# UltronAI/Depth-VO-Feat

Hardware: AMD Instinct MI355X
Metric: KITTI 256x832 stereo-seq samples/sec fwd+bwd (higher is better)
Workload: dtype f32

## Files before the change

### depth-vo-feat_amd/csrc/conv_head.hip

```cpp
#include "conv_head.h"
#include "conv_epilogue.h"

namespace {

using dvfp::apply_act;

constexpr int HT_W = 64, HT_H = 4;
constexpr int HP_W = HT_W + 2, HP_H = HT_H + 2;
constexpr int HCK = 8;

__device__ __forceinline__ void stage_tile(float *lds, const float *__restrict__ src, int64_t plane, int nch, int H, int W,
                                           int y0, int x0) {
    for (int e = threadIdx.x; e < nch * HP_H * HP_W; e += 256) {
        const int ch = e / (HP_H * HP_W), r = e - ch * (HP_H * HP_W), py = r / HP_W, px = r - py * HP_W;
        const int y = y0 + py - 1, x = x0 + px - 1;
        lds[e] = (y >= 0 && y < H && x >= 0 && x < W) ? src[ch * plane + (int64_t)y * W + x] : 0.f;
    }
}

template <int ROWS, int MO, class WK>
__device__ __forceinline__ void taps9(const float (&v)[ROWS + 2][3], WK wk, float (&acc)[ROWS][MO]) {
#pragma unroll
    for (int m = 0; m < MO; ++m)
#pragma unroll
        for (int k = 0; k < 9; ++k) {
            const float w = wk(m, k);
#pragma unroll
            for (int r = 0; r < ROWS; ++r) acc[r][m] = fmaf(w, v[k / 3 + r][k % 3], acc[r][m]);
        }
}

constexpr int FT_H = 8;
constexpr int HEAD_MAX_SEGS = 3;
struct HeadSegs {
    const float *p[HEAD_MAX_SEGS];
    int c[HEAD_MAX_SEGS];
    int n;
};
template <int MO, int HCKT, int FTH>
__global__ __launch_bounds__(256) void head_fwd_kernel(const HeadSegs in, const float *__restrict__ w,
                                                       const float *__restrict__ bias, float *__restrict__ out, int C, int H,
                                                       int W, int tilesX, int act, float alpha, float beta, int ws_m, int ws_c,
                                                       int flip, const float *__restrict__ mask) {
    constexpr int ROWS = FTH / 4, FPH = FTH + 2, FPN = FPH * HP_W, FLD = (FPN + 255) / 256;
    extern __shared__ __attribute__((aligned(16))) float wsh[];
    float *tile = wsh + ((MO * C * 9 + 3) & ~3);
    for (int e = threadIdx.x; e < MO * C * 9; e += 256) {
        const int m = e / (C * 9), r = e - m * (C * 9), c = r / 9, k = r - c * 9;
        const float wv = w[(int64_t)m * ws_m + (int64_t)c * ws_c + (flip ? 8 - k : k)];
        if (MO == 16) wsh[(c * MO + m) * 9 + k] = wv;
        else wsh[e] = wv;
    }
    const int n = blockIdx.y, tY = blockIdx.x / tilesX, tX = blockIdx.x - tY * tilesX;
    const int y0 = tY * FTH, x0 = tX * HT_W;
    const int lx = threadIdx.x & (HT_W - 1), ly = (threadIdx.x >> 6) * ROWS;
    const int64_t plane = (int64_t)H * W;
    int soff[FLD];
#pragma unroll
    for (int i = 0; i < FLD; ++i) {
        const int e = threadIdx.x + 256 * i, py = e / HP_W, px = e - py * HP_W;
        const int y = y0 + py - 1, x = x0 + px - 1;
        soff[i] = (e < FPN && y >= 0 && y < H && x >= 0 && x < W) ? y * W + x : -1;
    }
    float acc[ROWS][MO];
#pragma unroll
    for (int m = 0; m < MO; ++m)
#pragma unroll
        for (int r = 0; r < ROWS; ++r) acc[r][m] = bias ? bias[m] : 0.f;
    float stg[HCKT][FLD];
    static_assert(HEAD_MAX_SEGS == 3, "segment select below");
    auto seg_ptr = [&](int sg) { return sg == 0 ? in.p[0] : sg == 1 ? in.p[1] : in.p[2]; };
    auto seg_ch = [&](int sg) { return sg == 0 ? in.c[0] : sg == 1 ? in.c[1] : in.c[2]; };
    auto issue = [&](int sg, int cs) {
        const int sc = seg_ch(sg), nch = min(HCKT, sc - cs);
        const float *src = seg_ptr(sg) + ((int64_t)n * sc + cs) * plane;
#pragma unroll
        for (int ch = 0; ch < HCKT; ++ch)
#pragma unroll
            for (int i = 0; i < FLD; ++i) stg[ch][i] = (ch < nch && soff[i] >= 0) ? src[ch * plane + soff[i]] : 0.f;
    };
    issue(0, 0);
    int sg = 0, cs = 0, cg = 0;
    while (sg < in.n) {
        const int nch = min(HCKT, seg_ch(sg) - cs);
        int sg2 = sg, cs2 = cs + HCKT;
        if (cs2 >= seg_ch(sg)) { ++sg2; cs2 = 0; }
        __syncthreads();
#pragma unroll
        for (int ch = 0; ch < HCKT; ++ch)
#pragma unroll
            for (int i = 0; i < FLD; ++i) {
                const int e = threadIdx.x + 256 * i;
                if (e < FPN) tile[ch * FPN + e] = stg[ch][i];
            }
        __syncthreads();
        if (sg2 < in.n) issue(sg2, cs2);
        auto hood = [&](int ch, float (&v)[ROWS + 2][3]) __attribute__((always_inline)) {
            const float *t = tile + ch * FPN + ly * HP_W + lx;
#pragma unroll
            for (int a = 0; a < ROWS + 2; ++a)
#pragma unroll
                for (int b = 0; b < 3; ++b) v[a][b] = t[a * HP_W + b];
        };
        if constexpr (MO != 16) {
            auto wlds = [&](int c) __attribute__((always_inline)) {
                return [=](int m, int k) __attribute__((always_inline)) { return wsh[(m * C + c) * 9 + k]; };
            };
            float part[3][ROWS][MO];
#pragma unroll
            for (int q = 0; q < 3; ++q)
#pragma unroll
                for (int r = 0; r < ROWS; ++r)
#pragma unroll
                    for (int m = 0; m < MO; ++m) part[q][r][m] = 0.f;
            int ch = 0;
            for (; ch + 4 <= nch; ch += 4) {
                float v4[4][ROWS + 2][3];
#pragma unroll
                for (int q = 0; q < 4; ++q) hood(ch + q, v4[q]);
#pragma unroll
                for (int q = 0; q < 4; ++q)
#pragma unroll
                    for (int m = 0; m < MO; ++m) {
                        const float *wm = wsh + (m * C + cg + ch + q) * 9;
#pragma unroll
                        for (int k = 0; k < 9; ++k) {
                            const float wk = wm[k];
#pragma unroll
                            for (int r = 0; r < ROWS; ++r) {
                                if (q == 0) acc[r][m] = fmaf(wk, v4[q][k / 3 + r][k % 3], acc[r][m]);
                                else part[q - 1][r][m] = fmaf(wk, v4[q][k / 3 + r][k % 3], part[q - 1][r][m]);
                            }
                        }
                    }
            }
            for (; ch < nch; ++ch) {
                float v[ROWS + 2][3];
                hood(ch, v);
                taps9<ROWS, MO>(v, wlds(cg + ch), acc);
            }
#pragma unroll
            for (int r = 0; r < ROWS; ++r)
#pragma unroll
                for (int m = 0; m < MO; ++m) acc[r][m] += (part[0][r][m] + part[1][r][m]) + part[2][r][m];
        } else {
            for (int ch = 0; ch < nch; ++ch) {
                float v[ROWS + 2][3];
                hood(ch, v);
                typedef float f4h __attribute__((ext_vector_type(4)));
                const f4h *wq = reinterpret_cast<const f4h *>(wsh + (cg + ch) * (MO * 9));
                f4h wr[MO * 9 / 4];
#pragma unroll
                for (int q = 0; q < MO * 9 / 4; ++q) wr[q] = wq[q];
                taps9<ROWS, MO>(v, [&](int m, int k) __attribute__((always_inline)) { return wr[(m * 9 + k) >> 2][(m * 9 + k) & 3]; }, acc);
            }
        }
        cg += nch; sg = sg2; cs = cs2;
    }
    const int x = x0 + lx;
#pragma unroll
    for (int r = 0; r < ROWS; ++r) {
        const int y = y0 + ly + r;
        if (y < H && x < W) {
            if (mask) {
#pragma unroll
                for (int m = 0; m < MO; ++m) {
                    const int64_t idx = ((int64_t)n * MO + m) * plane + (int64_t)y * W + x;
                    out[idx] = mask[idx] > 0.f ? acc[r][m] : 0.f;
                }
            } else {
#pragma unroll
                for (int m = 0; m < MO; ++m)
                    out[((int64_t)n * MO + m) * plane + (int64_t)y * W + x] = apply_act(acc[r][m], act, alpha, beta);
            }
        }
    }
}

template <int MO>
__global__ __launch_bounds__(256) void head_dgrad_kernel(const float *__restrict__ dpre, const float *__restrict__ w,
                                                         float *__restrict__ din, int C, int H, int W, int tilesX,
                                                         const float *__restrict__ mask) {
    __shared__ float tile[MO * HP_H * HP_W];
    extern __shared__ __attribute__((aligned(16))) float wsh[];
    constexpr int WPC = (MO * 9 + 3) & ~3;
    for (int e = threadIdx.x; e < C * MO * 9; e += 256) {
        const int c = e / (MO * 9), r = e - c * (MO * 9), m = r / 9, k = r - m * 9;
        wsh[c * WPC + r] = w[((int64_t)m * C + c) * 9 + k];
    }
    const int n = blockIdx.y, tY = blockIdx.x / tilesX, tX = blockIdx.x - tY * tilesX;
    const int y0 = tY * HT_H, x0 = tX * HT_W;
    const int lx = threadIdx.x & (HT_W - 1), ly = threadIdx.x >> 6;
    const int64_t plane = (int64_t)H * W;
    stage_tile(tile, dpre + (int64_t)n * MO * plane, plane, MO, H, W, y0, x0);
    __syncthreads();
    float g[MO][9];
#pragma unroll
    for (int m = 0; m < MO; ++m)
#pragma unroll
        for (int a = 0; a < 3; ++a)
#pragma unroll
            for (int b = 0; b < 3; ++b) g[m][a * 3 + b] = tile[m * (HP_H * HP_W) + (ly + 2 - a) * HP_W + (lx + 2 - b)];
    const int y = y0 + ly, x = x0 + lx;
    if (y >= H || x >= W) return;
    const int64_t base = (int64_t)n * C * plane + (int64_t)y * W + x;
    float *dst = din + base;
    const float *mk = mask ? mask + base : nullptr;
    for (int c0 = 0; c0 < C; c0 += 4) {
        float sv[4], mv[4];
#pragma unroll
        for (int q = 0; q < 4; ++q) {
            const int c = min(c0 + q, C - 1);
            mv[q] = mk ? mk[c * plane] : 1.f;
            const float *wc = wsh + c * WPC;
            float s = 0.f;
#pragma unroll
            for (int m = 0; m < MO; ++m)
#pragma unroll
                for (int k = 0; k < 9; ++k) s = fmaf(wc[m * 9 + k], g[m][k], s);
            sv[q] = s;
        }
#pragma unroll
        for (int q = 0; q < 4; ++q)
            if (c0 + q < C) dst[(c0 + q) * plane] = (mv[q] > 0.f) ? sv[q] : 0.f;
    }
}

template <bool VEC>
__device__ __forceinline__ void hw_load4(const float *__restrict__ p, int x0, int W, bool ok, float (&v)[4]) {
    if (VEC) {
        typedef float f4 __attribute__((ext_vector_type(4)));
        f4 t = {0.f, 0.f, 0.f, 0.f};
        if (ok) t = *reinterpret_cast<const f4 *>(p);
#pragma unroll
        for (int j = 0; j < 4; ++j) v[j] = t[j];
    } else {
#pragma unroll
        for (int j = 0; j < 4; ++j) v[j] = (ok && x0 + j < W) ? p[j] : 0.f;
    }
}

template <int MO, int CCH, bool VEC>
__global__ __launch_bounds__(256) void head_wgrad_kernel(const float *__restrict__ in, const float *__restrict__ dpre,
                                                         float *dw, int C, int H, int W, int RS, int xgroups, int segs,
                                                         int64_t units, float *part = nullptr) {
    constexpr int A = CCH * 9 * MO;
    __shared__ float red[4 * A];
    const int c0 = blockIdx.x * CCH;
    const int64_t plane = (int64_t)H * W;
    const int upi = segs * xgroups;
    float acc[CCH][9][MO];
#pragma unroll
    for (int c = 0; c < CCH; ++c)
#pragma unroll
        for (int t = 0; t < 9; ++t)
#pragma unroll
            for (int m = 0; m < MO; ++m) acc[c][t][m] = 0.f;
    for (int64_t ub = blockIdx.y; ub * 256 < units; ub += gridDim.y) {
        const int64_t u = ub * 256 + threadIdx.x;
        const bool live = u < units;
        const int n = live ? (int)(u / upi) : 0, q = live ? (int)(u - (int64_t)n * upi) : 0;
        const int seg = q / xgroups, xg = q - seg * xgroups;
        const int y0 = seg * RS, y1 = min(H, y0 + RS), x0 = xg * 4;
        const float *ip = in + ((int64_t)n * C + c0) * plane + x0;
        const float *dp = dpre + (int64_t)n * MO * plane + x0;
        const bool lok = x0 > 0, rok = x0 + 4 < W;
        auto load_in = [&](int r, float (&x)[CCH][6]) __attribute__((always_inline)) {
            const bool ok = live && r >= 0 && r < H;
            const int64_t ro = (int64_t)r * W;
#pragma unroll
            for (int c = 0; c < CCH; ++c) {
                const bool okc = ok && c0 + c < C;
                const float *p = ip + c * plane + ro;
                float v[4];
                hw_load4<VEC>(p, x0, W, okc, v);
                x[c][0] = (okc && lok) ? p[-1] : 0.f;
#pragma unroll
                for (int j = 0; j < 4; ++j) x[c][1 + j] = v[j];
                x[c][5] = (okc && rok) ? p[4] : 0.f;
            }
        };
        auto load_dp = [&](int y, float (&g)[MO][4]) __attribute__((always_inline)) {
            const bool ok = live && y >= y0 && y < y1;
#pragma unroll
            for (int m = 0; m < MO; ++m) hw_load4<VEC>(dp + m * plane + (int64_t)y * W, x0, W, ok, g[m]);
        };
        float d[3][MO][4], dn[MO][4], xc[CCH][6], xn[CCH][6];
#pragma unroll
        for (int m = 0; m < MO; ++m)
#pragma unroll
            for (int j = 0; j < 4; ++j) d[0][m][j] = d[1][m][j] = 0.f;
        load_dp(y0, d[2]);
        load_in(y0 - 1, xc);
        for (int i = 0; i < RS + 2; ++i) {
            const int r = y0 - 1 + i;
            load_in(i + 1 < RS + 2 ? r + 1 : H, xn);
            load_dp(r + 2, dn);
#pragma unroll
            for (int c = 0; c < CCH; ++c)
#pragma unroll
                for (int ta = 0; ta < 3; ++ta)
#pragma unroll
                    for (int tb = 0; tb < 3; ++tb)
#pragma unroll
                        for (int m = 0; m < MO; ++m)
#pragma unroll
                            for (int j = 0; j < 4; ++j)
                                acc[c][ta * 3 + tb][m] = fmaf(d[2 - ta][m][j], xc[c][j + tb], acc[c][ta * 3 + tb][m]);
#pragma unroll
            for (int m = 0; m < MO; ++m)
#pragma unroll
                for (int j = 0; j < 4; ++j) { d[0][m][j] = d[1][m][j]; d[1][m][j] = d[2][m][j]; d[2][m][j] = dn[m][j]; }
#pragma unroll
            for (int c = 0; c < CCH; ++c)
#pragma unroll
                for (int j = 0; j < 6; ++j) xc[c][j] = xn[c][j];
        }
    }
    const int wave = threadIdx.x >> 6, lane = threadIdx.x & 63;
#pragma unroll
    for (int c = 0; c < CCH; ++c)
#pragma unroll
        for (int t = 0; t < 9; ++t)
#pragma unroll
            for (int m = 0; m < MO; ++m) {
                const float s = wave_sum(acc[c][t][m]);
                if (lane == 0) red[wave * A + (c * 9 + t) * MO + m] = s;
            }
    __syncthreads();
    const int a = threadIdx.x;
    if (a < A) {
        const int c = a / (9 * MO), q = a - c * (9 * MO), t = q / MO, m = q - t * MO;
        if (c0 + c < C) {
            const float s = (red[a] + red[A + a]) + (red[2 * A + a] + red[3 * A + a]);
            const int64_t o = ((int64_t)m * C + c0 + c) * 9 + t;
            if (part) part[(int64_t)blockIdx.y * MO * C * 9 + o] = s;
            else atomicAdd(&dw[o], s);
        }
    }
}

__global__ __launch_bounds__(256) void head_wgrad_finish_kernel(const float *__restrict__ part, float *dw, int n, int groups) {
    const int e = blockIdx.x * 256 + threadIdx.x;
    if (e >= n) return;
    float s = 0.f;
    for (int g = 0; g < groups; ++g) s += part[(int64_t)g * n + e];
    dw[e] += s;
}


template <int CO, int K>
__global__ __launch_bounds__(256) void dconvt_s2_fwd_kernel(const float *__restrict__ in, const float *__restrict__ w,
                                                            const float *__restrict__ bias, float *__restrict__ out, int C, int H,
                                                            int W, int OH, int OW, int act, float alpha, float beta) {
    extern __shared__ __attribute__((aligned(16))) float wlds[];
    constexpr int WPC = CO * K * K;
    static_assert(WPC % 4 == 0, "weights of one input channel are read in 16-byte pieces");
    typedef float f4w __attribute__((ext_vector_type(4)));
    for (int e = threadIdx.x; e < C * WPC / 4; e += 256)
        reinterpret_cast<f4w *>(wlds)[e] = reinterpret_cast<const f4w *>(w)[e];
    __syncthreads();
    const int x = blockIdx.x * 64 + (threadIdx.x & 63), y = blockIdx.y * 4 + (threadIdx.x >> 6), n = blockIdx.z;
    const bool inside = x < W && y < H;
    const bool rok[3] = {y - 1 >= 0 && y - 1 < H, y < H, y + 1 < H}, cok[3] = {x - 1 >= 0 && x - 1 < W, x < W, x + 1 < W};
    float acc[2][2][CO];
#pragma unroll
    for (int co = 0; co < CO; ++co) {
        const float b = bias ? bias[co] : 0.f;
        acc[0][0][co] = acc[0][1][co] = acc[1][0][co] = acc[1][1][co] = b;
    }
    const int64_t plane = (int64_t)H * W;
    const float *ip = in + (int64_t)n * C * plane + (int64_t)y * W + x;
    for (int ci = 0; ci < C; ++ci) {
        float v[3][3];
#pragma unroll
        for (int r = (K == 3 ? 1 : 0); r < 3; ++r)
#pragma unroll
            for (int c = (K == 3 ? 1 : 0); c < 3; ++c) v[r][c] = (rok[r] && cok[c]) ? ip[(r - 1) * W + (c - 1)] : 0.f;
        const f4w *wc = reinterpret_cast<const f4w *>(wlds + ci * WPC);
        f4w wq[WPC / 4];
#pragma unroll
        for (int q = 0; q < WPC / 4; ++q) wq[q] = wc[q];
#pragma unroll
        for (int co = 0; co < CO; ++co) {
#pragma unroll
            for (int a = 0; a < K; ++a) {
                const int dy = (a + 1) & 1;
                const int ry = 1 + ((dy + 1 - a) >> 1);
#pragma unroll
                for (int b = 0; b < K; ++b) {
                    const int dx = (b + 1) & 1;
                    const int rx = 1 + ((dx + 1 - b) >> 1);
                    const int f = co * K * K + a * K + b;
                    acc[dy][dx][co] = fmaf(wq[f >> 2][f & 3], v[ry][rx], acc[dy][dx][co]);
                }
            }
        }
        ip += plane;
    }
    if (!inside) return;
    const int64_t oplane = (int64_t)OH * OW;
    float *op = out + (int64_t)n * CO * oplane;
#pragma unroll
    for (int dy = 0; dy < 2; ++dy) {
        const int Y = 2 * y + dy;
        if (Y >= OH) continue;
        const int X = 2 * x;
#pragma unroll
        for (int co = 0; co < CO; ++co) {
            float r0 = apply_act(acc[dy][0][co], act, alpha, beta), r1 = apply_act(acc[dy][1][co], act, alpha, beta);
            float *q = op + co * oplane + (int64_t)Y * OW + X;
            if (X + 1 < OW && (OW & 1) == 0) {
                typedef float f2 __attribute__((ext_vector_type(2)));
                f2 t; t.x = r0; t.y = r1;
                *reinterpret_cast<f2 *>(q) = t;
            } else {
                if (X < OW) q[0] = r0;
                if (X + 1 < OW) q[1] = r1;
            }
        }
    }
}

}

bool dvf_head_applicable(const dvf_conv_desc *d, int nseg) {
    return nseg == 1 && !d->transposed && d->KH == 3 && d->KW == 3 && d->stride == 1 && d->pad == 1 && d->C_out >= 1 &&
           d->C_out <= 4 && d->H_out == d->H_in && d->W_out == d->W_in && d->C_in >= 4 && d->C_in * d->C_out <= 1024 &&
           dvf_tune("DVF_NO_HEAD") == nullptr;
}
bool dvf_head_fwd_applicable(const dvf_conv_desc *d, int nseg) {
    static const int maxc = dvf_tune("DVF_HEAD_FWD_MAXC") ? atoi(dvf_tune("DVF_HEAD_FWD_MAXC")) : 127;
    return dvf_head_applicable(d, nseg) && d->C_in <= maxc;
}
bool dvf_head_dgrad_applicable(const dvf_conv_desc *d, int nseg) {
    static const int maxc = dvf_tune("DVF_HEAD_DGRAD_MAXC") ? atoi(dvf_tune("DVF_HEAD_DGRAD_MAXC")) : 32;
    return dvf_head_applicable(d, nseg) && d->C_in <= maxc;
}

bool dvf_dconvt_applicable(const dvf_conv_desc *d, int nseg) {
    const bool k3 = d->KH == 3 && d->KW == 3, k4 = d->KH == 4 && d->KW == 4;
    return nseg == 1 && d->transposed && d->stride == 2 && d->pad == 1 && (k3 || k4) && d->C_out == 16 &&
           d->C_in >= 8 && d->C_in <= 64 && d->H_out <= 2 * d->H_in && d->W_out <= 2 * d->W_in &&
           (int64_t)d->H_in * d->W_in >= 64 * 64 && (int64_t)d->N * d->C_out * d->H_out * d->W_out < ((int64_t)1 << 31) &&
           dvf_tune("DVF_NO_DCONVT") == nullptr;
}

int dvf_dconvt_fwd(const dvf_conv_desc *d, const float *in, const float *w, const float *bias, float *out, hipStream_t st) {
    const dim3 grid(cdiv(d->W_in, 64), cdiv(d->H_in, 4), d->N);
    const size_t lds = (size_t)d->C_in * d->C_out * d->KH * d->KW * 4;
    if ((reinterpret_cast<uintptr_t>(w) & 15) != 0 || lds > 64 * 1024) return DVF_ERR_UNSUPPORTED;
#define DCONVT(CO, K) dconvt_s2_fwd_kernel<CO, K><<<grid, 256, lds, st>>>(in, w, bias, out, d->C_in, d->H_in, d->W_in, d->H_out, d->W_out, d->act, d->alpha, d->beta)
    if (d->KH == 3) DCONVT(16, 3);
    else DCONVT(16, 4);
#undef DCONVT
    DVF_LAUNCH_CHECK();
    dvf_note_head(DVF_K_DCONVT_FWD, d->C_out, d->KH);
    return DVF_OK;
}

#define HEAD_CASE(N, ...) case N: { constexpr int MO = N; __VA_ARGS__; } break;
#define HEAD_DISPATCH(MOV, CALL, ...)             \
    switch (MOV) {                               \
        HEAD_CASE(1, CALL) HEAD_CASE(2, CALL) HEAD_CASE(3, CALL) HEAD_CASE(4, CALL) __VA_ARGS__ \
        default: return DVF_ERR_UNSUPPORTED;     \
    }

static int head_fwd_launch(int MOv, const HeadSegs &in, const float *w, const float *bias, float *out, int C, int N, int H, int W,
                           int act, float alpha, float beta, int ws_m, int ws_c, int flip, const float *mask, hipStream_t st) {
    const bool lowres = (int64_t)N * H * W <= (int64_t)4 * 64 * 208 && MOv <= 4 && C >= 32;
    const int FTH = lowres ? 4 : FT_H, HCKT = lowres ? 32 : HCK;
    const int tilesX = cdiv(W, HT_W), tilesY = cdiv(H, FTH);
    const dim3 grid(tilesX * tilesY, N);
    const size_t lds = ((size_t)((MOv * C * 9 + 3) & ~3) + (size_t)HCKT * (FTH + 2) * HP_W) * 4;
#define HEAD_FWD_GO(HC, FH) head_fwd_kernel<MO, HC, FH><<<grid, 256, lds, st>>>(in, w, bias, out, C, H, W, tilesX, act, alpha, beta, ws_m, ws_c, flip, mask)
    if (lowres) {
        static bool big[5] = {false, false, false, false, false};
        HEAD_DISPATCH(MOv, {
            if (lds > 64 * 1024 && !big[MO]) {
                if (hipFuncSetAttribute(reinterpret_cast<const void *>(&head_fwd_kernel<MO, 32, 4>), hipFuncAttributeMaxDynamicSharedMemorySize, 160 * 1024) != hipSuccess) return DVF_ERR_LAUNCH;
                big[MO] = true;
            }
            HEAD_FWD_GO(32, 4); });
    } else {
        HEAD_DISPATCH(MOv, (HEAD_FWD_GO(8, 8)), HEAD_CASE(16, (HEAD_FWD_GO(8, 8))));
    }
#undef HEAD_FWD_GO
    DVF_LAUNCH_CHECK();
    return DVF_OK;
}

int dvf_head_fwd(const dvf_conv_desc *d, const float *in, const float *w, const float *bias, float *out, hipStream_t st) {
    const int one = d->C_in;
    return dvf_head_fwd_segs(d, &in, &one, 1, w, bias, out, st);
}

bool dvf_head_wide_applicable(const dvf_conv_desc *d, int nseg) {
    return nseg >= 1 && nseg <= HEAD_MAX_SEGS && !d->transposed && d->KH == 3 && d->KW == 3 && d->stride == 1 && d->pad == 1 &&
           d->C_out == 16 && d->C_in <= 24 && d->H_out == d->H_in && d->W_out == d->W_in &&
           (int64_t)d->H_in * d->W_in >= 64 * 64 && dvf_tune("DVF_NO_HEAD") == nullptr && dvf_tune("DVF_NO_WIDE_HEAD") == nullptr;
}

int dvf_head_fwd_segs(const dvf_conv_desc *d, const float *const *in_segs, const int *seg_channels, int nseg, const float *w,
                      const float *bias, float *out, hipStream_t st) {
    HeadSegs in{};
    for (int s = 0; s < HEAD_MAX_SEGS; ++s) { in.p[s] = s < nseg ? in_segs[s] : in_segs[0]; in.c[s] = s < nseg ? seg_channels[s] : 0; }
    in.n = nseg;
    const int rc = head_fwd_launch(d->C_out, in, w, bias, out, d->C_in, d->N, d->H_in, d->W_in, d->act, d->alpha, d->beta,
                                   d->C_in * 9, 9, 0, nullptr, st);
    if (rc) return rc;
    dvf_note_head(DVF_K_HEAD_FWD, d->C_out, nseg);
    return DVF_OK;
}

bool dvf_head_seg_dgrad_applicable(const dvf_conv_desc *d, int segc) {
    const bool narrow = segc >= 1 && segc <= 4 && d->C_out >= 4 && d->C_out * segc <= 1024;
    const bool wide = segc == 16 && d->C_out <= 24 && (int64_t)d->H_in * d->W_in >= 64 * 64 &&
                      dvf_tune("DVF_NO_WIDE_HEAD") == nullptr;
    return !d->transposed && d->KH == 3 && d->KW == 3 && d->stride == 1 && d->pad == 1 && (narrow || wide) &&
           d->H_out == d->H_in && d->W_out == d->W_in && dvf_tune("DVF_NO_HEAD") == nullptr;
}

int dvf_head_seg_dgrad(const dvf_conv_desc *d, const float *dpre, const float *w, float *din, int seg_off, int segc,
                       hipStream_t st, const float *mask) {
    const float *wseg = w + (int64_t)seg_off * 9;
    HeadSegs in{};
    for (int s = 0; s < HEAD_MAX_SEGS; ++s) { in.p[s] = dpre; in.c[s] = s == 0 ? d->C_out : 0; }
    in.n = 1;
    const int rc = head_fwd_launch(segc, in, wseg, nullptr, din, d->C_out, d->N, d->H_in, d->W_in, DVF_ACT_NONE, 1.f, 0.f, 9,
                                   d->C_in * 9, 1, mask, st);
    if (rc) return rc;
    dvf_note_head(DVF_K_HEAD_SEG_DGRAD, segc);
    return DVF_OK;
}

int dvf_head_dgrad(const dvf_conv_desc *d, const float *dpre, const float *w, float *din, hipStream_t st, const float *mask) {
    const int tilesX = cdiv(d->W_in, HT_W), tilesY = cdiv(d->H_in, HT_H);
    const dim3 grid(tilesX * tilesY, d->N);
    HEAD_DISPATCH(d->C_out, (head_dgrad_kernel<MO><<<grid, 256, (size_t)d->C_in * ((MO * 9 + 3) & ~3) * 4, st>>>(
                                dpre, w, din, d->C_in, d->H_in, d->W_in, tilesX, mask)));
    DVF_LAUNCH_CHECK();
    dvf_note_head(DVF_K_HEAD_DGRAD, d->C_out);
    return DVF_OK;
}

struct HeadWgradGrid { int cch, RS, xgroups, segs, chunks, groups; int64_t units; };
static HeadWgradGrid head_wgrad_grid(const dvf_conv_desc *d) {
    HeadWgradGrid g;
    g.xgroups = cdiv(d->W_in, 4);
    auto blocks = [&](int cch, int rs) {
        return (int64_t)cdiv(d->C_in, cch) * (((int64_t)d->N * cdiv(d->H_in, rs) * g.xgroups + 255) / 256);
    };
    const int min_blocks = 400, max_blocks = 1024;
    g.cch = (d->C_out <= 2 && blocks(4, 8) >= 512) ? 4 : 2;
    g.RS = 8;
    if (const char *t = dvf_tune("DVF_HEAD_WG_CCH")) g.cch = (atoi(t) == 4 && d->C_out <= 2) ? 4 : 2;
    while (g.RS > 2 && blocks(g.cch, g.RS) < min_blocks) g.RS >>= 1;
    if (const char *t = dvf_tune("DVF_HEAD_WG_RS")) g.RS = atoi(t) > 0 ? atoi(t) : g.RS;
    g.segs = cdiv(d->H_in, g.RS);
    g.units = (int64_t)d->N * g.segs * g.xgroups;
    g.chunks = cdiv(d->C_in, g.cch);
    const int64_t nub = (g.units + 255) / 256;
    int64_t groups = max_blocks / g.chunks;
    if (groups < 1) groups = 1;
    if (groups > nub) groups = nub;
    g.groups = (int)groups;
    return g;
}

int64_t dvf_head_wgrad_ws_floats(const dvf_conv_desc *d) {
    return (int64_t)head_wgrad_grid(d).groups * d->C_out * d->C_in * 9;
}

int dvf_head_wgrad(const dvf_conv_desc *d, const float *in, const float *dpre, float *dw, int accumulate, hipStream_t st,
                   float *ws, int64_t ws_floats) {
    if (!accumulate && hipMemsetAsync(dw, 0, sizeof(float) * (size_t)d->C_out * d->C_in * 9, st) != hipSuccess)
        return DVF_ERR_LAUNCH;
    const HeadWgradGrid g = head_wgrad_grid(d);
    const dim3 grid(g.chunks, g.groups);
    float *part = (ws && ws_floats >= dvf_head_wgrad_ws_floats(d)) ? ws : nullptr;
    const bool vec = d->W_in % 4 == 0 && ((reinterpret_cast<uintptr_t>(in) | reinterpret_cast<uintptr_t>(dpre)) & 15) == 0;
#define HEAD_WGRAD_GO(CCH, VEC) head_wgrad_kernel<MO, CCH, VEC><<<grid, 256, 0, st>>>(in, dpre, dw, d->C_in, d->H_in, d->W_in, g.RS, g.xgroups, g.segs, g.units, part)
    HEAD_DISPATCH(d->C_out, {
        if (MO <= 2 && g.cch == 4) { if (vec) HEAD_WGRAD_GO((MO <= 2 ? 4 : 2), true); else HEAD_WGRAD_GO((MO <= 2 ? 4 : 2), false); }
        else { if (vec) HEAD_WGRAD_GO(2, true); else HEAD_WGRAD_GO(2, false); } });
#undef HEAD_WGRAD_GO
    DVF_LAUNCH_CHECK();
    if (part) {
        const int n = d->C_out * d->C_in * 9;
        head_wgrad_finish_kernel<<<(n + 255) / 256, 256, 0, st>>>(part, dw, n, g.groups);
        DVF_LAUNCH_CHECK();
    }
    dvf_note_head(DVF_K_HEAD_WGRAD, d->C_out, part != nullptr);
    return DVF_OK;
}
```

Before: 663.5.

## Add MFMA kernels for stride-2 transposed conv and thin 16-output 3x3 conv

Adds an MFMA (16x16x4 f32 matrix-core) version of the stride-2 transposed convolution. It decomposes the output into four parity classes and double-buffers input and weight chunks through registers into LDS. It also adds a persistent-block MFMA kernel for 3x3 convolutions with 16 outputs and at most 24 input channels, which prefetches the next tile while computing the current one. The transposed-conv path is on by default when C_in is a multiple of 4, while the thin 3x3 path runs only when DVF_THIN_MFMA=1. The goal is to move the scalar FMA work onto matrix cores, at the cost of extra LDS staging and more code complexity.

```diff
diff --git a/depth-vo-feat_amd/csrc/conv_head.hip b/depth-vo-feat_amd/csrc/conv_head.hip
--- a/depth-vo-feat_amd/csrc/conv_head.hip
+++ b/depth-vo-feat_amd/csrc/conv_head.hip
@@ -422,6 +422,274 @@
     }
 }
 
+typedef float f4m __attribute__((ext_vector_type(4)));
+constexpr int TM_W = 64, TM_H = 4, TM_RS = TM_W + 2, TM_PN = (TM_H + 2) * TM_RS, TM_FLD = (TM_PN + 255) / 256;
+
+constexpr int T3_PS = TM_PN + 10;
+constexpr int T3_WLD = (24 * 9 * 16 + 255) / 256;
+constexpr int T3_BLOCKS = 4 * 256;
+template <int SC>
+__global__ __launch_bounds__(256) void thin3x3_mfma_kernel(const HeadSegs in, const float *__restrict__ w,
+                                                           const float *__restrict__ bias, float *__restrict__ out, int C, int H,
+                                                           int W, int tilesX, int tilesY, int total, int act, float alpha, float beta,
+                                                           int ws_m, int ws_c, int flip, const float *__restrict__ mask) {
+    extern __shared__ __attribute__((aligned(16))) float wsh[];
+    const int K = C * 9, NS = (K + 3) >> 2;
+    float *tile = wsh + NS * 64;
+    const int lane = threadIdx.x & 63, wave = threadIdx.x >> 6, g = lane >> 4, px = lane & 15;
+    const int64_t plane = (int64_t)H * W;
+    const int per = tilesX * tilesY;
+    static_assert(HEAD_MAX_SEGS == 3, "segment select below");
+    const int c01 = in.c[0] + in.c[1];
+    int soff[TM_FLD];
+    float stg[SC][TM_FLD];
+    auto issue = [&](int t) {
+        const int n = t / per, r = t - n * per, tY = r / tilesX, tX = r - tY * tilesX;
+#pragma unroll
+        for (int i = 0; i < TM_FLD; ++i) {
+            const int e = threadIdx.x + 256 * i, py = e / TM_RS, qx = e - py * TM_RS;
+            const int y = tY * TM_H + py - 1, x = tX * TM_W + qx - 1;
+            soff[i] = (e < TM_PN && y >= 0 && y < H && x >= 0 && x < W) ? y * W + x : -1;
+        }
+#pragma unroll
+        for (int ch = 0; ch < SC; ++ch) {
+            const int c = min(ch, C - 1), sg = (c >= in.c[0]) + (c >= c01);
+            const float *sp = sg == 0 ? in.p[0] : sg == 1 ? in.p[1] : in.p[2];
+            const int sc = sg == 0 ? in.c[0] : sg == 1 ? in.c[1] : in.c[2], first = sg == 0 ? 0 : sg == 1 ? in.c[0] : c01;
+            const float *src = sp + ((int64_t)n * sc + (c - first)) * plane;
+#pragma unroll
+            for (int i = 0; i < TM_FLD; ++i) stg[ch][i] = src[max(soff[i], 0)];
+        }
+    };
+    {
+        float wst[T3_WLD];
+#pragma unroll
+        for (int i = 0; i < T3_WLD; ++i) {
+            const int e = threadIdx.x + 256 * i, k = min(e >> 4, K - 1), m = e & 15, c = k / 9, t = k - c * 9;
+            wst[i] = 256 * i < NS * 64 ? w[(int64_t)m * ws_m + (int64_t)c * ws_c + (flip ? 8 - t : t)] : 0.f;
+        }
+        issue(blockIdx.x);
+#pragma unroll
+        for (int i = 0; i < T3_WLD; ++i) {
+            const int e = threadIdx.x + 256 * i;
+            if (e < NS * 64) wsh[e] = (e >> 4) < K ? wst[i] : 0.f;
+        }
+        if (C & 3)
+            for (int e = threadIdx.x; e < TM_PN; e += 256) tile[C * T3_PS + e] = 0.f;
+    }
+    int boff[9];
+#pragma unroll
+    for (int s = 0; s < 9; ++s) {
+        const int kl = 4 * s + g, cl = kl / 9, t = kl - cl * 9;
+        boff[s] = cl * T3_PS + (t / 3) * TM_RS + (t % 3);
+    }
+    float bv[4];
+#pragma unroll
+    for (int r = 0; r < 4; ++r) bv[r] = bias ? bias[4 * g + r] : 0.f;
+    for (int t = blockIdx.x; t < total; t += gridDim.x) {
+        __syncthreads();
+#pragma unroll
+        for (int ch = 0; ch < SC; ++ch)
+#pragma unroll
+            for (int i = 0; i < TM_FLD; ++i) {
+                const int e = threadIdx.x + 256 * i;
+                if (ch < C && e < TM_PN) tile[ch * T3_PS + e] = soff[i] >= 0 ? stg[ch][i] : 0.f;
+            }
+        __syncthreads();
+        if (t + (int)gridDim.x < total) issue(t + gridDim.x);
+        f4m acc[4];
+#pragma unroll
+        for (int r = 0; r < 4; ++r)
+#pragma unroll
+            for (int q = 0; q < 4; ++q) acc[q][r] = bv[r];
+        const float *tb = tile + wave * TM_RS + px, *wb = wsh + lane;
+        int s0 = 0;
+        for (; s0 + 9 <= NS; s0 += 9) {
+#pragma unroll
+            for (int s3 = 0; s3 < 9; s3 += 3) {
+                float a[3], b[3][4];
+#pragma unroll
+                for (int s = 0; s < 3; ++s) {
+                    a[s] = wb[(s3 + s) * 64];
+#pragma unroll
+                    for (int q = 0; q < 4; ++q) b[s][q] = tb[boff[s3 + s] + 16 * q];
+                }
+                __builtin_amdgcn_sched_barrier(0);
+#pragma unroll
+                for (int s = 0; s < 3; ++s)
+#pragma unroll
+                    for (int q = 0; q < 4; ++q) acc[q] = __builtin_amdgcn_mfma_f32_16x16x4f32(a[s], b[s][q], acc[q], 0, 0, 0);
+                __builtin_amdgcn_sched_barrier(0);
+            }
+            tb += 4 * T3_PS;
+            wb += 9 * 64;
+        }
+#pragma unroll
+        for (int s = 0; s < 8; ++s)
+            if (s0 + s < NS) {
+                const float a = wb[s * 64];
+                float b[4];
+#pragma unroll
+                for (int q = 0; q < 4; ++q) b[q] = tb[boff[s] + 16 * q];
+#pragma unroll
+                for (int q = 0; q < 4; ++q) acc[q] = __builtin_amdgcn_mfma_f32_16x16x4f32(a, b[q], acc[q], 0, 0, 0);
+            }
+        const int n = t / per, rt = t - n * per, tY = rt / tilesX, tX = rt - tY * tilesX;
+        const int y = tY * TM_H + wave, x0 = tX * TM_W;
+        if (y >= H) continue;
+        const int64_t row = ((int64_t)n * 16 + 4 * g) * plane + (int64_t)y * W;
+        if (mask) {
+            float mv[4][4];
+#pragma unroll
+            for (int q = 0; q < 4; ++q)
+#pragma unroll
+                for (int r = 0; r < 4; ++r) mv[q][r] = mask[row + r * plane + min(x0 + 16 * q + px, W - 1)];
+#pragma unroll
+            for (int q = 0; q < 4; ++q)
+#pragma unroll
+                for (int r = 0; r < 4; ++r) acc[q][r] = mv[q][r] > 0.f ? acc[q][r] : 0.f;
+        } else {
+#pragma unroll
+            for (int q = 0; q < 4; ++q)
+#pragma unroll
+                for (int r = 0; r < 4; ++r) acc[q][r] = apply_act(acc[q][r], act, alpha, beta);
+        }
+#pragma unroll
+        for (int q = 0; q < 4; ++q) {
+            const int x = x0 + 16 * q + px;
+            if (x >= W) continue;
+#pragma unroll
+            for (int r = 0; r < 4; ++r) out[row + r * plane + x] = acc[q][r];
+        }
+    }
+}
+
+constexpr int TT_PS = TM_PN + 4;
+constexpr int TT_CS = 8;
+__host__ __device__ constexpr int dct_ntap(int K, int d) { return (K == 3 && d == 0) ? 1 : 2; }
+__host__ __device__ constexpr int dct_tap(int d, int j) { return (d == 0 ? 1 : 0) + 2 * j; }
+__host__ __device__ constexpr int dct_src(int d, int a) { return 1 + ((d + 1 - a) >> 1); }
+template <int K>
+__global__ __launch_bounds__(256) void dconvt_s2_mfma_kernel(const float *__restrict__ in, const float *__restrict__ w,
+                                                             const float *__restrict__ bias, float *__restrict__ out, int C, int H,
+                                                             int W, int OH, int OW, int act, float alpha, float beta) {
+    constexpr int KK = K * K, WS = KK | 1, CW = 16 * WS;
+    constexpr int WN = TT_CS * 16 * KK, WLD = (WN + 255) / 256;
+    __shared__ float tile[TT_CS * TT_PS];
+    __shared__ float wl[TT_CS * CW];
+    const int lane = threadIdx.x & 63, wave = threadIdx.x >> 6, g = lane >> 4, px = lane & 15;
+    const int x0 = blockIdx.x * TM_W, y0 = blockIdx.y * TM_H, n = blockIdx.z;
+    const int64_t plane = (int64_t)H * W;
+    int soff[TM_FLD];
+#pragma unroll
+    for (int i = 0; i < TM_FLD; ++i) {
+        const int e = threadIdx.x + 256 * i, py = e / TM_RS, qx = e - py * TM_RS;
+        const int y = y0 + py - 1, x = x0 + qx - 1;
+        soff[i] = (e < TM_PN && y >= 0 && y < H && x >= 0 && x < W) ? y * W + x : -1;
+    }
+    int boff[4], aoff[4];
+#pragma unroll
+    for (int cls = 0; cls < 4; ++cls) {
+        const int dy = cls >> 1, dx = cls & 1, nb = dct_ntap(K, dx), T = dct_ntap(K, dy) * nb;
+        const int cil = g / T, t = g - cil * T, a = dct_tap(dy, t / nb), b = dct_tap(dx, t % nb);
+        boff[cls] = cil * TT_PS + dct_src(dy, a) * TM_RS + dct_src(dx, b);
+        aoff[cls] = (cil * 16 + px) * WS + a * K + b;
+    }
+    f4m acc[4][4];
+#pragma unroll
+    for (int r = 0; r < 4; ++r) {
+        const float bv = bias ? bias[4 * g + r] : 0.f;
+#pragma unroll
+        for (int cls = 0; cls < 4; ++cls)
+#pragma unroll
+            for (int q = 0; q < 4; ++q) acc[cls][q][r] = bv;
+    }
+    const float *ip = in + (int64_t)n * C * plane;
+    float stg[TT_CS][TM_FLD], wst[WLD];
+    auto issue = [&](int c0) {
+#pragma unroll
+        for (int ch = 0; ch < TT_CS; ++ch) {
+            const float *src = ip + min(c0 + ch, C - 1) * plane;
+#pragma unroll
+            for (int i = 0; i < TM_FLD; ++i) stg[ch][i] = src[max(soff[i], 0)];
+        }
+        const int wlim = min(WN, (C - c0) * 16 * KK);
+#pragma unroll
+        for (int i = 0; i < WLD; ++i) wst[i] = w[(int64_t)c0 * 16 * KK + min((int)threadIdx.x + 256 * i, wlim - 1)];
+    };
+    issue(0);
+    const float *tb = tile + wave * TM_RS + px;
+    for (int c0 = 0; c0 < C; c0 += TT_CS) {
+        __syncthreads();
+#pragma unroll
+        for (int ch = 0; ch < TT_CS; ++ch)
+#pragma unroll
+            for (int i = 0; i < TM_FLD; ++i) {
+                const int e = threadIdx.x + 256 * i;
+                if (e < TM_PN) tile[ch * TT_PS + e] = soff[i] >= 0 ? stg[ch][i] : 0.f;
+            }
+#pragma unroll
+        for (int i = 0; i < WLD; ++i) {
+            const int e = threadIdx.x + 256 * i;
+            if (e < WN) wl[e + (e / KK) * (WS - KK)] = wst[i];
+        }
+        __syncthreads();
+        if (c0 + TT_CS < C) issue(c0 + TT_CS);
+        const int nper = min(TT_CS, C - c0) >> 2;
+        for (int pp = 0; pp < nper; ++pp) {
+            const float *tp = tb + pp * 4 * TT_PS, *wp = wl + pp * 4 * CW;
+#pragma unroll
+            for (int cls = 0; cls < 4; ++cls) {
+                const int T = dct_ntap(K, cls >> 1) * dct_ntap(K, cls & 1);
+                float a[4], b[4][4];
+#pragma unroll
+                for (int i = 0; i < 4; ++i)
+                    if (i < T) {
+                        const int cstep = i * (4 / T);
+                        a[i] = wp[aoff[cls] + cstep * CW];
+#pragma unroll
+                        for (int q = 0; q < 4; ++q) b[i][q] = tp[boff[cls] + cstep * TT_PS + 16 * q];
+                    }
+                __builtin_amdgcn_sched_barrier(0);
+#pragma unroll
+                for (int i = 0; i < 4; ++i)
+                    if (i < T) {
+#pragma unroll
+                        for (int q = 0; q < 4; ++q)
+                            acc[cls][q] = __builtin_amdgcn_mfma_f32_16x16x4f32(a[i], b[i][q], acc[cls][q], 0, 0, 0);
+                    }
+            }
+        }
+    }
+    const int y = y0 + wave;
+    if (y >= H) return;
+    const int64_t oplane = (int64_t)OH * OW;
+    float *op = out + (int64_t)n * 16 * oplane;
+#pragma unroll
+    for (int q = 0; q < 4; ++q) {
+        const int x = x0 + 16 * q + px, X = 2 * x;
+        if (x >= W) continue;
+#pragma unroll
+        for (int dy = 0; dy < 2; ++dy) {
+            const int Y = 2 * y + dy;
+            if (Y >= OH) continue;
+#pragma unroll
+            for (int r = 0; r < 4; ++r) {
+                const float r0 = apply_act(acc[dy * 2][q][r], act, alpha, beta), r1 = apply_act(acc[dy * 2 + 1][q][r], act, alpha, beta);
+                float *o = op + (4 * g + r) * oplane + (int64_t)Y * OW + X;
+                if (X + 1 < OW && (OW & 1) == 0) {
+                    typedef float f2 __attribute__((ext_vector_type(2)));
+                    f2 t; t.x = r0; t.y = r1;
+                    *reinterpret_cast<f2 *>(o) = t;
+                } else {
+                    if (X < OW) o[0] = r0;
+                    if (X + 1 < OW) o[1] = r1;
+                }
+            }
+        }
+    }
+}
+
 }
 
 bool dvf_head_applicable(const dvf_conv_desc *d, int nseg) {
@@ -446,13 +714,25 @@
            dvf_tune("DVF_NO_DCONVT") == nullptr;
 }
 
+static int thin_mfma_knob() {
+    const char *e = dvf_tune("DVF_THIN_MFMA");
+    return e ? (atoi(e) != 0) : -1;
+}
+
 int dvf_dconvt_fwd(const dvf_conv_desc *d, const float *in, const float *w, const float *bias, float *out, hipStream_t st) {
     const dim3 grid(cdiv(d->W_in, 64), cdiv(d->H_in, 4), d->N);
     const size_t lds = (size_t)d->C_in * d->C_out * d->KH * d->KW * 4;
     if ((reinterpret_cast<uintptr_t>(w) & 15) != 0 || lds > 64 * 1024) return DVF_ERR_UNSUPPORTED;
-#define DCONVT(CO, K) dconvt_s2_fwd_kernel<CO, K><<<grid, 256, lds, st>>>(in, w, bias, out, d->C_in, d->H_in, d->W_in, d->H_out, d->W_out, d->act, d->alpha, d->beta)
-    if (d->KH == 3) DCONVT(16, 3);
-    else DCONVT(16, 4);
+    static_assert(TM_W == 64 && TM_H == 4, "both forms run the same grid");
+    const bool mfma = d->C_in % 4 == 0 && thin_mfma_knob() != 0;
+#define DCONVT(LDS, ...) __VA_ARGS__<<<grid, 256, LDS, st>>>(in, w, bias, out, d->C_in, d->H_in, d->W_in, d->H_out, d->W_out, d->act, d->alpha, d->beta)
+    if (mfma) {
+        if (d->KH == 3) DCONVT(0, dconvt_s2_mfma_kernel<3>);
+        else DCONVT(0, dconvt_s2_mfma_kernel<4>);
+    } else {
+        if (d->KH == 3) DCONVT(lds, dconvt_s2_fwd_kernel<16, 3>);
+        else DCONVT(lds, dconvt_s2_fwd_kernel<16, 4>);
+    }
 #undef DCONVT
     DVF_LAUNCH_CHECK();
     dvf_note_head(DVF_K_DCONVT_FWD, d->C_out, d->KH);
@@ -468,6 +748,19 @@
 
 static int head_fwd_launch(int MOv, const HeadSegs &in, const float *w, const float *bias, float *out, int C, int N, int H, int W,
                            int act, float alpha, float beta, int ws_m, int ws_c, int flip, const float *mask, hipStream_t st) {
+    if (MOv == 16 && C <= 24 && thin_mfma_knob() == 1) {
+        const int tilesX = cdiv(W, TM_W), tilesY = cdiv(H, TM_H), NS = (C * 9 + 3) >> 2, planes = C + ((C & 3) ? 1 : 0);
+        const int64_t total = (int64_t)tilesX * tilesY * N;
+        if (total >= ((int64_t)1 << 31)) return DVF_ERR_UNSUPPORTED;
+        const size_t lds = ((size_t)NS * 64 + (size_t)planes * T3_PS) * 4;
+        const int blocks = (int)(total < T3_BLOCKS ? total : T3_BLOCKS);
+#define THIN3_GO(SC) thin3x3_mfma_kernel<SC><<<blocks, 256, lds, st>>>(in, w, bias, out, C, H, W, tilesX, tilesY, (int)total, act, alpha, beta, ws_m, ws_c, flip, mask)
+        if (C <= 18) THIN3_GO(18);
+        else THIN3_GO(24);
+#undef THIN3_GO
+        DVF_LAUNCH_CHECK();
+        return DVF_OK;
+    }
     const bool lowres = (int64_t)N * H * W <= (int64_t)4 * 64 * 208 && MOv <= 4 && C >= 32;
     const int FTH = lowres ? 4 : FT_H, HCKT = lowres ? 32 : HCK;
     const int tilesX = cdiv(W, HT_W), tilesY = cdiv(H, FTH);
```

Result: no change. 664.1, median of 4 (+0.1%).
